# vliu15/3d-brain-tumor-segmentation

Measured on AMD Instinct MI355X. Metric: training volumes/sec (2ch x 128^3), higher is better.
Workload: dtype f32; 1 GPU; BASELINE configs[1]: 2ch x 128^3, batch 1 per GPU, fp32, full fwd+bwd with Dice+KL+L2 VAE loss + Dice metric + TF-form Adam; CLI-default model (base_filters=32, depth=4, groups=8, reduction=8; 42,174,773 params); parallelism=dp1, global_batch=1

## Files before the change

3d-brain-tumor-segmentation_amd/csrc/conv_igemm.hip:

```cpp
#include <stdlib.h>
#include "common.h"
#include "bts_internal.h"

#define MAXSLOT 8

int bts_prof_on();
void bts_prof_begin(int sym, double flops, hipStream_t stream);
void bts_prof_end(hipStream_t stream);

struct IgemmParams {
  const float* x;
  const float* wp;
  const float* bias;
  float* y;
  int N, Di, Hi, Wi, Cin, ldx;
  int Do, Ho, Wo;
  int Cout, ldy, Npad, KG;
  int ODa, OHa, OWa;
  int os, ooz, ooy, oox;
  int s, loz, loy, lox;
  int IZ, IY, IX;
  int lgTX, lgTY, TZ;
  int ntz, nty, ntx;
  int ntaps, flags;
// ... 943 lines not shown
  if (need > 0 && (ws == nullptr || ws_bytes < need)) return 1;
  p.x = x; p.wp = wp; p.bias = bias; p.y = y; p.ldx = ldx; p.ldy = ldy; p.flags = flags;
  p.part = reinterpret_cast<float*>(ws);
  const long tiles = (long)N * p.ntz * p.nty * p.ntx;
  const int ny = p.Npad / 32;
  const int tileVox = p.IZ * p.IY * p.IX;
  const size_t shmem = (size_t)2 * tileVox * 12 * sizeof(float);
  const bool prof = bts_prof_on();
  if (prof) bts_prof_begin(20, 2.0 * 27.0 * Cin * Cout * (double)N * Di * Hi * Wi, stream);
  (void)hipGetLastError(); hipLaunchKernelGGL(upm_kernel, dim3((unsigned)tiles, ny, p.ksplit), dim3(256), shmem, stream, p);
  if (prof) bts_prof_end(stream);
  BTS_LAUNCH_CHECK();
  if (p.ksplit > 1) {
    const long nvox = (long)N * 8 * Di * Hi * Wi;
    long blocks = (nvox * Cout + 255) / 256;
    if (blocks > 4096) blocks = 4096;
    (void)hipGetLastError(); hipLaunchKernelGGL(igemm_reduce_kernel, dim3((int)blocks), dim3(256), 0, stream, p.part, bias, y, nvox, Cout, p.Npad, ldy,
                       p.ksplit, flags);
    BTS_LAUNCH_CHECK();
  }
  return BTS_OK;
}

struct K1sParams {
  const float* x;
  const float* wp;
  const float* bias;
  float* y;
  long nvox;
  int Cin, ldx, Cout, ldy, Npad, KG, flags;
};
template <int NS>
__global__ __launch_bounds__(256, 4) void k1s_kernel(const K1sParams p) {
  const int lane = threadIdx.x & 63;
  const int wave = __builtin_amdgcn_readfirstlane(threadIdx.x >> 6);
  const int h = lane >> 5, l32 = lane & 31;
  const long v0 = (long)blockIdx.x * 256 + wave * 64;
  const float* xrow[2];
#pragma unroll
  for (int ms = 0; ms < 2; ++ms) {
    long v = v0 + ms * 32 + l32;
    if (v >= p.nvox) v = p.nvox - 1;
    xrow[ms] = p.x + v * p.ldx + h * 4;
  }
  int woff[NS];
#pragma unroll
  for (int ns = 0; ns < NS; ++ns) {
    int ncol = (blockIdx.y * NS + ns) * 32 + l32;
    if (ncol >= p.Npad) ncol = p.Npad - 1;
    woff[ns] = (h * p.Npad + ncol) * 4;
  }
  const int wstepKG = 2 * p.Npad * 4;
  f32x16 acc[2][NS];
#pragma unroll
  for (int ms = 0; ms < 2; ++ms)
#pragma unroll
    for (int ns = 0; ns < NS; ++ns)
#pragma unroll
      for (int r = 0; r < 16; ++r) acc[ms][ns][r] = 0.f;
  constexpr int U = (NS == 1) ? 2 : 1;
  f32x4 b[2][U][2], a[2][U][NS];
  auto load = [&](int buf, int kg) {
#pragma unroll
    for (int u = 0; u < U; ++u) {
      const int k = (kg + u < p.KG) ? kg + u : p.KG - 1;
#pragma unroll
      for (int ms = 0; ms < 2; ++ms) b[buf][u][ms] = *reinterpret_cast<const f32x4*>(xrow[ms] + k * 8);
#pragma unroll
      for (int ns = 0; ns < NS; ++ns) a[buf][u][ns] = *reinterpret_cast<const f32x4*>((p.wp + k * wstepKG) + woff[ns]);
    }
  };
  auto mma = [&](int buf, int kg) {
#pragma unroll
    for (int u = 0; u < U; ++u) {
      if (kg + u < p.KG) {
#pragma unroll
        for (int j = 0; j < 4; ++j)
#pragma unroll
          for (int ms = 0; ms < 2; ++ms)
#pragma unroll
            for (int ns = 0; ns < NS; ++ns)
              acc[ms][ns] = __builtin_amdgcn_mfma_f32_32x32x2f32(a[buf][u][ns][j], b[buf][u][ms][j], acc[ms][ns], 0, 0, 0);
      }
    }
  };
  load(0, 0);
  for (int kg = 0; kg < p.KG; kg += 2 * U) {
    if (kg + U < p.KG) load(1, kg + U);
    mma(0, kg);
    if (kg + U < p.KG) {
      if (kg + 2 * U < p.KG) load(0, kg + 2 * U);
      mma(1, kg + U);
    }
  }
#pragma unroll
  for (int ms = 0; ms < 2; ++ms) {
    const long v = v0 + ms * 32 + l32;
    if (v >= p.nvox) continue;
    float* yrow = p.y + v * p.ldy;
#pragma unroll
    for (int ns = 0; ns < NS; ++ns) {
      const int nb = (blockIdx.y * NS + ns) * 32;
#pragma unroll
      for (int g = 0; g < 4; ++g) {
        const int co = nb + 8 * g + 4 * h;
        if (co >= p.Cout) continue;
        f32x4 val = {acc[ms][ns][4 * g + 0], acc[ms][ns][4 * g + 1], acc[ms][ns][4 * g + 2], acc[ms][ns][4 * g + 3]};
        if (p.flags & IG_FLAG_BIAS) {
#pragma unroll
          for (int j = 0; j < 4; ++j)
            if (co + j < p.Cout) val[j] += p.bias[co + j];
        }
        if (p.flags & IG_FLAG_SIGMOID) {
#pragma unroll
          for (int j = 0; j < 4; ++j) val[j] = sigmoidf_(val[j]);
        }
        if ((p.flags & IG_FLAG_VECOUT) && co + 3 < p.Cout) {
          f32x4* dst = reinterpret_cast<f32x4*>(yrow + co);
          if (p.flags & IG_FLAG_ACCUM) val += *dst;
          *dst = val;
        } else {
#pragma unroll
          for (int j = 0; j < 4; ++j)
            if (co + j < p.Cout) yrow[co + j] = (p.flags & IG_FLAG_ACCUM) ? yrow[co + j] + val[j] : val[j];
        }
      }
    }
  }
}

static int launch_k1s(const float* x, const float* wp, const float* bias, float* y, long nvox, int Cin, int ldx, int Cout, int ldy,
                      int flags, hipStream_t stream) {
  if ((Cin & 7) || (ldx & 3) || (((uintptr_t)x) & 15)) return 1;
  const long min_vox = getenv("BTS_IGEMM_K1S_MIN") ? atol(getenv("BTS_IGEMM_K1S_MIN")) : 256 * 256;
  if (nvox < min_vox) return 1;
  K1sParams p;
  p.x = x; p.wp = wp; p.bias = bias; p.y = y; p.nvox = nvox;
  p.Cin = Cin; p.ldx = ldx; p.Cout = Cout; p.ldy = ldy; p.Npad = npad32(Cout); p.KG = Cin / 8;
  p.flags = flags & (IG_FLAG_BIAS | IG_FLAG_ACCUM | IG_FLAG_SIGMOID);
  if ((ldy % 4 == 0) && (((uintptr_t)y) % 16 == 0)) p.flags |= IG_FLAG_VECOUT;
  const long gx = (nvox + 255) / 256;
  if (gx > 0x7fffffffL) return 1;
  const bool prof = bts_prof_on();
  const int ns = (p.Npad >= 64) ? 2 : 1;
  if (prof) bts_prof_begin(21, 2.0 * Cin * (double)Cout * (double)nvox, stream);
  (void)hipGetLastError();
  if (ns == 2) hipLaunchKernelGGL(k1s_kernel<2>, dim3((unsigned)gx, (p.Npad + 63) / 64), dim3(256), 0, stream, p);
  else hipLaunchKernelGGL(k1s_kernel<1>, dim3((unsigned)gx, 1), dim3(256), 0, stream, p);
  if (prof) bts_prof_end(stream);
  BTS_LAUNCH_CHECK();
  return BTS_OK;
}

struct DscParams {
  const float* x;
  const float* wp;
  const float* bias;
  float* y;
  int N, D, H, W, Cin, ldx, Cout, ldy, Npad, KG, ntx, nty, ntz, flags;
};
template <int CO>
__global__ __launch_bounds__(256, 4) void dsc_kernel(const DscParams p) {
  constexpr int S = 12, TX = 32, TY = 4, TZ = 2, IX = TX + 2, IY = TY + 2, IZ = TZ + 2;
  constexpr int tileVox = IZ * IY * IX, nslots = tileVox * 2, NSL = (nslots + 255) / 256;
  __shared__ __attribute__((aligned(16))) float lds[tileVox * S];
  const int tid = threadIdx.x;
  int b = blockIdx.x;
  const int tx = b % p.ntx; b /= p.ntx;
  const int ty = b % p.nty; b /= p.nty;
  const int tz = b % p.ntz;
  const int n = b / p.ntz;
  const int iz0 = tz * TZ - 1, iy0 = ty * TY - 1, ix0 = tx * TX - 1;
  const float* xbase = p.x + ((((long)n * p.D + iz0) * p.H + iy0) * p.W + ix0) * (long)p.ldx;
  int goff[NSL];
#pragma unroll
  for (int i = 0; i < NSL; ++i) {
    const int e = tid + i * 256;
    goff[i] = -1;
    if (e < nslots) {
      const int vox = e >> 1, q = e & 1;
      const int vz = vox / (IY * IX), r = vox - vz * (IY * IX), vy = r / IX, vx = r - vy * IX;
      if ((unsigned)(iz0 + vz) < (unsigned)p.D && (unsigned)(iy0 + vy) < (unsigned)p.H && (unsigned)(ix0 + vx) < (unsigned)p.W)
        goff[i] = ((vz * p.H + vy) * p.W + vx) * p.ldx + q * 4;
    }
  }
  const int mx = tid & (TX - 1), my = (tid >> 5) & (TY - 1), mz = tid >> 7;
  const float* lb = lds + ((mz * IY + my) * IX + mx) * S;
  float acc[CO];
#pragma unroll
  for (int c = 0; c < CO; ++c) acc[c] = 0.f;
  const int wstepKG = 2 * p.Npad * 4, wstepTap = p.KG * wstepKG;
  f32x4 pre[NSL];
  auto fetch = [&](int kg) {
#pragma unroll
    for (int i = 0; i < NSL; ++i) {
      f32x4 v = {0.f, 0.f, 0.f, 0.f};
      if (goff[i] >= 0) v = *reinterpret_cast<const f32x4*>(xbase + goff[i] + kg * 8);
      pre[i] = v;
    }
  };
  fetch(0);
  for (int kg = 0; kg < p.KG; ++kg) {
    __syncthreads();
#pragma unroll
    for (int i = 0; i < NSL; ++i) {
      const int e = tid + i * 256;
      if (e < nslots) *reinterpret_cast<f32x4*>(lds + (e >> 1) * S + (e & 1) * 4) = pre[i];
    }
    __syncthreads();
    if (kg + 1 < p.KG) fetch(kg + 1);
    const float* wk = p.wp + kg * wstepKG;
#pragma unroll
    for (int r = 0; r < 9; ++r) {
      float w[3][2][CO * 4];
#pragma unroll
      for (int dx = 0; dx < 3; ++dx)
#pragma unroll
        for (int hh = 0; hh < 2; ++hh)
#pragma unroll
          for (int q = 0; q < CO * 4; ++q) w[dx][hh][q] = wk[(r * 3 + dx) * wstepTap + hh * p.Npad * 4 + q];
      f32x4 xv[3][2];
#pragma unroll
      for (int dx = 0; dx < 3; ++dx) {
        const float* src = lb + (((r / 3) * IY + r % 3) * IX + dx) * S;
        xv[dx][0] = *reinterpret_cast<const f32x4*>(src);
        xv[dx][1] = *reinterpret_cast<const f32x4*>(src + 4);
      }
      __builtin_amdgcn_sched_barrier(0);
#pragma unroll
      for (int dx = 0; dx < 3; ++dx)
#pragma unroll
        for (int hh = 0; hh < 2; ++hh)
#pragma unroll
          for (int c = 0; c < CO; ++c)
#pragma unroll
            for (int j = 0; j < 4; ++j) acc[c] = fmaf(xv[dx][hh][j], w[dx][hh][c * 4 + j], acc[c]);
      __builtin_amdgcn_sched_barrier(0);
    }
  }
  const int oz = tz * TZ + mz, oy = ty * TY + my, ox = tx * TX + mx;
  if (oz >= p.D || oy >= p.H || ox >= p.W) return;
  float* yrow = p.y + ((((long)n * p.D + oz) * p.H + oy) * p.W + ox) * (long)p.ldy;
#pragma unroll
  for (int c = 0; c < CO; ++c) {
    if (c < p.Cout) {
      float v = acc[c];
      if (p.flags & IG_FLAG_BIAS) v += p.bias[c];
      if (p.flags & IG_FLAG_SIGMOID) v = sigmoidf_(v);
      if (p.flags & IG_FLAG_ACCUM) v += yrow[c];
      yrow[c] = v;
    }
  }
}

static int launch_dsc(const float* x, const float* wp, const float* bias, float* y, int N, int D, int H, int W, int Cin, int ldx,
                      int Cout, int ldy, int flags, hipStream_t stream) {
  if (Cout > 4 || (Cin & 7) || (ldx & 3) || (((uintptr_t)x) & 15)) return 1;
  const long tiles = (long)N * ((D + 1) / 2) * ((H + 3) / 4) * ((W + 31) / 32);
  const long min_tiles = getenv("BTS_IGEMM_DSC_MIN") ? atol(getenv("BTS_IGEMM_DSC_MIN")) : 1024;
  if (tiles < min_tiles || tiles > 0x7fffffffL) return 1;
  DscParams p;
  p.x = x; p.wp = wp; p.bias = bias; p.y = y;
  p.N = N; p.D = D; p.H = H; p.W = W; p.Cin = Cin; p.ldx = ldx; p.Cout = Cout; p.ldy = ldy;
  p.Npad = npad32(Cout); p.KG = Cin / 8;
  p.ntx = (W + 31) / 32; p.nty = (H + 3) / 4; p.ntz = (D + 1) / 2;
  p.flags = flags & (IG_FLAG_BIAS | IG_FLAG_ACCUM | IG_FLAG_SIGMOID);
  const bool prof = bts_prof_on();
  if (prof) bts_prof_begin(22, 2.0 * 27.0 * Cin * (double)Cout * (double)N * D * H * W, stream);
  (void)hipGetLastError();
  if (Cout <= 2) hipLaunchKernelGGL(dsc_kernel<2>, dim3((unsigned)tiles), dim3(256), 0, stream, p);
  else hipLaunchKernelGGL(dsc_kernel<4>, dim3((unsigned)tiles), dim3(256), 0, stream, p);
  if (prof) bts_prof_end(stream);
  BTS_LAUNCH_CHECK();
  return BTS_OK;
}

struct C2Params {
  const float* x;
  const float* wp;
  const float* bias;
  float* y;
  const float* wp2;
  const float* bias2;
  float* y2;
  int N, D, H, W, ldx, Cout, ldy, ldy2, Npad;
  int ntz, nty, ntx;
  double* gnp;
  int gn_G, gn_zt;
};

template <bool F2>
__global__ __launch_bounds__(256, 2) void c2_kernel(const C2Params p) {
  __shared__ float lds[2 * 6 * 6 * 34 + 16];
  const int tid = threadIdx.x;
  const int lane = tid & 63;
  const int wave = __builtin_amdgcn_readfirstlane(tid >> 6);
  const int h = lane >> 5, l32 = lane & 31;
  int b = blockIdx.x;
  const int tx = b % p.ntx; b /= p.ntx;
  const int ty = b % p.nty; b /= p.nty;
  const int tz = b % p.ntz;
  const int n = b / p.ntz;
  const int oz0 = tz * 4, oy0 = ty * 4, ox0 = tx * 32;
  for (int e = tid; e < 6 * 6 * 34; e += 256) {
    const int vz = e / (6 * 34), r = e - vz * (6 * 34);
    const int vy = r / 34, vx = r - vy * 34;
    const int z = oz0 - 1 + vz, yy = oy0 - 1 + vy, xx = ox0 - 1 + vx;
    float v0 = 0.f, v1 = 0.f;
    if ((unsigned)z < (unsigned)p.D && (unsigned)yy < (unsigned)p.H && (unsigned)xx < (unsigned)p.W) {
      const float* s = p.x + ((((long)n * p.D + z) * p.H + yy) * p.W + xx) * (long)p.ldx;
      v0 = s[0]; v1 = s[1];
    }
    lds[e] = v0;
    lds[6 * 6 * 34 + e] = v1;
  }
  float wt[27];
#pragma unroll
  for (int t = 0; t < 27; ++t) wt[t] = p.wp[((long)t * 2 * p.Npad + l32) * 4 + h];
  float w2 = 0.f;
  if (F2) w2 = p.wp2[l32 * 4 + h];
  __syncthreads();
  f32x16 acc[4], acc2[F2 ? 4 : 1];
#pragma unroll
  for (int i = 0; i < 4; ++i)
#pragma unroll
    for (int r = 0; r < 16; ++r) { acc[i][r] = 0.f; if (F2) acc2[F2 ? i : 0][r] = 0.f; }
  const float* lb = lds + h * (6 * 6 * 34) + (wave * 6) * 34 + l32;
#pragma unroll
  for (int kz = 0; kz < 3; ++kz) {
    float f[6][3];
#pragma unroll
    for (int yr = 0; yr < 6; ++yr)
#pragma unroll
      for (int kx = 0; kx < 3; ++kx) f[yr][kx] = lb[(kz * 6 + yr) * 34 + kx];
#pragma unroll
    for (int ky = 0; ky < 3; ++ky)
#pragma unroll
      for (int kx = 0; kx < 3; ++kx)
#pragma unroll
        for (int oy = 0; oy < 4; ++oy)
          acc[oy] = __builtin_amdgcn_mfma_f32_32x32x2f32(wt[(kz * 3 + ky) * 3 + kx], f[oy + ky][kx], acc[oy], 0, 0, 0);
    if (F2 && kz == 1) {
#pragma unroll
      for (int oy = 0; oy < 4; ++oy) acc2[F2 ? oy : 0] = __builtin_amdgcn_mfma_f32_32x32x2f32(w2, f[oy + 1][1], acc2[F2 ? oy : 0], 0, 0, 0);
    }
  }
  const int oz = oz0 + wave, ox = ox0 + l32;
  float gn_s = 0.f, gn_q = 0.f;
  if (oz < p.D && ox < p.W) {
#pragma unroll
    for (int oy = 0; oy < 4; ++oy) {
      const int y = oy0 + oy;
      if (y >= p.H) continue;
      const long pix = (((long)n * p.D + oz) * p.H + y) * p.W + ox;
#pragma unroll
      for (int g = 0; g < 4; ++g) {
        const int co = 8 * g + 4 * h;
        if (co >= p.Cout) continue;
        f32x4 v = {acc[oy][4 * g], acc[oy][4 * g + 1], acc[oy][4 * g + 2], acc[oy][4 * g + 3]};
        if (p.bias) {
#pragma unroll
          for (int j = 0; j < 4; ++j) v[j] += p.bias[co + j];
        }
        if (p.gnp) {
#pragma unroll
          for (int j = 0; j < 4; ++j) { gn_s += v[j]; gn_q = fmaf(v[j], v[j], gn_q); }
        }
        *reinterpret_cast<f32x4*>(p.y + pix * p.ldy + co) = v;
        if (F2) {
          f32x4 v2 = {acc2[F2 ? oy : 0][4 * g], acc2[F2 ? oy : 0][4 * g + 1], acc2[F2 ? oy : 0][4 * g + 2], acc2[F2 ? oy : 0][4 * g + 3]};
          if (p.bias2) {
#pragma unroll
            for (int j = 0; j < 4; ++j) v2[j] += p.bias2[co + j];
          }
          *reinterpret_cast<f32x4*>(p.y2 + pix * p.ldy2 + co) = v2;
        }
      }
    }
  }
  if (p.gnp) {
    const double ds = wave_sum_f64((double)gn_s), dq = wave_sum_f64((double)gn_q);
    __syncthreads();
    double* sh = reinterpret_cast<double*>(lds);
    if (lane == 0) { sh[wave * 2] = ds; sh[wave * 2 + 1] = dq; }
    __syncthreads();
    if (tid == 0) {
      const int g = tz / p.gn_zt;
      const long B = (long)p.gn_zt * p.nty * p.ntx;
      const long b_ = ((long)(tz - g * p.gn_zt) * p.nty + ty) * p.ntx + tx;
      double* o = p.gnp + (((long)n * p.gn_G + g) * B + b_) * 2;
      o[0] = sh[0] + sh[2] + sh[4] + sh[6];
      o[1] = sh[1] + sh[3] + sh[5] + sh[7];
    }
  }
}

static int launch_c2(const float* x, const float* wp, const float* bias, float* y, int N, int D, int H, int W, int Cin, int ldx,
                     int Cout, int ldy, int flags, const float* wp2, const float* bias2, float* y2, int ldy2, double* gnp, int gnG,
                     long* gn_B, hipStream_t stream) {
  if (Cin != 2 || Cout > 32 || Cout % 4 != 0 || ldy % 4 != 0 || (((uintptr_t)y) & 15)) return 1;
  if (flags & (IG_FLAG_ACCUM | IG_FLAG_SIGMOID)) return 1;
  if (y2 != nullptr && (ldy2 % 4 != 0 || (((uintptr_t)y2) & 15))) return 1;
  C2Params p;
  p.x = x; p.wp = wp; p.bias = (flags & IG_FLAG_BIAS) ? bias : nullptr; p.y = y;
  p.wp2 = wp2; p.bias2 = bias2; p.y2 = y2;
  p.N = N; p.D = D; p.H = H; p.W = W; p.ldx = ldx; p.Cout = Cout; p.ldy = ldy; p.ldy2 = ldy2; p.Npad = npad32(Cout);
  p.ntz = (D + 3) / 4; p.nty = (H + 3) / 4; p.ntx = (W + 31) / 32;
  const long tiles = (long)N * p.ntz * p.nty * p.ntx;
  const long min_tiles = getenv("BTS_IGEMM_C2_MIN") ? atol(getenv("BTS_IGEMM_C2_MIN")) : 512;
  if (tiles < min_tiles || tiles > 0x7fffffffL) return 1;
  p.gnp = nullptr; p.gn_G = 0; p.gn_zt = 1;
  if (gnp != nullptr && gnG > 0 && D % gnG == 0 && (D / gnG) % 4 == 0 && getenv("BTS_IGEMM_NOGNFUSE") == nullptr) {
    p.gnp = gnp; p.gn_G = gnG; p.gn_zt = (D / gnG) / 4;
  }
  const bool prof = bts_prof_on();
  if (prof) bts_prof_begin(25, 2.0 * (27.0 + (y2 ? 1.0 : 0.0)) * Cin * (double)Cout * (double)N * D * H * W, stream);
  (void)hipGetLastError();
  if (y2 != nullptr) hipLaunchKernelGGL(c2_kernel<true>, dim3((unsigned)tiles), dim3(256), 0, stream, p);
  else hipLaunchKernelGGL(c2_kernel<false>, dim3((unsigned)tiles), dim3(256), 0, stream, p);
  if (prof) bts_prof_end(stream);
  BTS_LAUNCH_CHECK();
  if (gn_B && p.gnp != nullptr) *gn_B = (long)p.gn_zt * p.nty * p.ntx;
  return BTS_OK;
}

enum Geo { GEO_K1 = 0, GEO_S1 = 1, GEO_DOWN = 2, GEO_UP = 3 };

template <int MS, int NS, int WM, int WN, int KGS, bool FUSE2 = false, bool FIXG = false, bool T27 = false>
static int launch_cfg(IgemmParams& p, hipStream_t stream) {
  constexpr int S = KGS * 8 + 4;
  const int tileVox = p.IZ * p.IY * p.IX;
  if (tileVox * KGS * 2 > 256 * MAXSLOT) return BTS_ERR_SHAPE;
  const int nstages_all = (p.KG + KGS - 1) / KGS;
  const size_t shmem = (size_t)((nstages_all > 1 && !IG_TRI(MS, NS, KGS, FUSE2, FIXG)) ? 2 : 1) * tileVox * S * sizeof(float);
  auto kern = igemm_kernel<MS, NS, WM, WN, KGS, FUSE2, FIXG, T27>;
  static bool attr_done = false;
  if (!attr_done && !p.plan_only) {
    hipError_t e = hipFuncSetAttribute(reinterpret_cast<const void*>(kern), hipFuncAttributeMaxDynamicSharedMemorySize, 160 * 1024);
    if (e != hipSuccess) return (int)e;
    attr_done = true;
  }
  const int NT = 32 * NS * WN;
  dim3 grid(p.N * p.ntz * p.nty * p.ntx, (p.Npad + NT - 1) / NT, p.ncls > 1 ? p.ncls : 1);
  p.ksplit = 1;
  p.kg_per = p.KG;
  p.ws_need = 0;
  const long wgs = (long)grid.x * grid.y;
  const long sk_below = (KGS == 1) ? 512 : 192, sk_target = (KGS == 1) ? 512 : 384;
  if (!FUSE2 && p.ncls <= 1 && wgs < sk_below && p.KG >= 4 * KGS) {
    int ks = (int)((sk_target + wgs - 1) / wgs);
    const int maxks = p.KG / (2 * KGS);
    if (ks > maxks) ks = maxks;
    if (ks > 64) ks = 64;
    if (ks > 1) {
      int per = (p.KG + ks - 1) / ks;
      per = (per + KGS - 1) / KGS * KGS;
      ks = (p.KG + per - 1) / per;
      const long need = (long)ks * p.N * p.Do * p.Ho * p.Wo * p.Npad * 4;
      if (ks > 1 && (p.plan_only || (p.part != nullptr && p.ws_bytes >= need))) {
        p.ksplit = ks;
        p.kg_per = per;
        p.ws_need = need;
        grid.z = ks;
      }
    }
  }
  if (p.ksplit > 1) p.gnp = nullptr;
  p.gn_gridy = (int)grid.y;
  if (p.plan_only) return BTS_OK;
  const bool prof = bts_prof_on();
  if (prof) {
    constexpr int cfgid = (MS == 2 && NS == 1) ? 0 : (MS == 2 && NS == 2) ? 1 : (MS == 1 && NS == 2) ? 2 : (WN == 2) ? 3 : 4;
    const double taps = (p.ncls > 1) ? 27.0 : (double)p.ntaps;
    bts_prof_begin(cfgid + (KGS == 4 ? 8 : 0), 2.0 * taps * p.Cin * p.Cout * (double)p.N * p.Do * p.Ho * p.Wo, stream);
  }
  (void)hipGetLastError(); hipLaunchKernelGGL(kern, grid, dim3(256), shmem, stream, p);
  if (prof) bts_prof_end(stream);
  BTS_LAUNCH_CHECK();
  if (p.ksplit > 1) {
    const long nvox = (long)p.N * p.Do * p.Ho * p.Wo;
    long blocks = (nvox * p.Cout + 255) / 256;
    if (blocks > 4096) blocks = 4096;
    (void)hipGetLastError(); hipLaunchKernelGGL(igemm_reduce_kernel, dim3((int)blocks), dim3(256), 0, stream, p.part, p.bias, p.y, nvox, p.Cout,
                       p.Npad, p.ldy, p.ksplit, p.flags);
    BTS_LAUNCH_CHECK();
  }
  return BTS_OK;
}

static int ilog2(int v) { int l = 0; while ((1 << l) < v) ++l; return l; }

static int choose_cfg(int geo, int N, int Do, int Ho, int Wo, int Npad, int* Mout) {
  const long vox = (long)Do * Ho * Wo;
  int M, cfg;
  if (geo == GEO_DOWN) {
    M = 64;
    cfg = (Npad >= 128) ? 2 : 3;
  } else {
    const long wg256 = (long)N * ((vox + 255) / 256) * ((Npad + 63) / 64);
    if (Npad <= 32) {
      if ((long)N * ((vox + 255) / 256) >= 512) { M = 256; cfg = 0; }
      else { M = 128; cfg = 4; }
    } else if (wg256 >= 512) { M = 256; cfg = 1; }
    else {
      M = 64;
      const long wg64_128 = (long)N * ((vox + 63) / 64) * ((Npad + 127) / 128);
      cfg = (Npad >= 128 && wg64_128 >= 384) ? 2 : 3;
    }
  }
  *Mout = M;
  return cfg;
}

static int launch_igemm(int geo, const float* x, const float* wp, const float* bias, float* y, int N, int Di, int Hi,
                        int Wi, int Cin, int ldx, int Do, int Ho, int Wo, int Cout, int ldy, int ODa, int OHa, int OWa,
                        int pz, int py, int px, int flags, hipStream_t stream, void* ws = nullptr, long ws_bytes = 0,
                        long* need_out = nullptr, const float* wp2 = nullptr, const float* bias2 = nullptr,
                        float* y2 = nullptr, int ldy2 = 0, double* gnp = nullptr, int gnG = 0, long* gn_B = nullptr,
                        const float* x2 = nullptr, int ldx2 = 0) {
  if (gn_B) *gn_B = 0;
  if (geo == GEO_S1 && wp2 == nullptr && need_out == nullptr && Cout <= 4) {
    { const int e = bts_img_ensure_(wp, 1u, stream); if (e != BTS_OK) return e; }
    const int r = launch_dsc(x, wp, bias, y, N, Di, Hi, Wi, Cin, ldx, Cout, ldy, flags, stream);
    if (r != 1) { bts_img_mark_used_(wp, 1u); return r; }
  }
  if (geo == GEO_S1 && need_out == nullptr && Cin == 2 && x2 == nullptr && (wp2 == nullptr) == (y2 == nullptr)) {
    { const int e = bts_img_ensure_(wp, 1u, stream); if (e != BTS_OK) return e; }
    const int r = launch_c2(x, wp, bias, y, N, Di, Hi, Wi, Cin, ldx, Cout, ldy, flags, wp2, bias2, y2, ldy2, gnp, gnG, gn_B, stream);
    if (r != 1) { bts_img_mark_used_(wp, 1u); return r; }
  }
  if (geo == GEO_S1 && need_out == nullptr && !(flags & IG_FLAG_SIGMOID)) {
    const long pairs = (long)((Cin + 7) / 8) * 2 * npad32(Cout) * 4;
    const float* up = wp + 27L * pairs;
    int r = bts_w3_launch_(x, up + 48L * pairs, (flags & IG_FLAG_BIAS) ? bias : nullptr, y, N, Di, Hi, Wi, Cin, ldx, Cout, ldy,
                           (flags & IG_FLAG_ACCUM) ? 1 : 0, gnp, gnG, gn_B, ws, ws_bytes, stream);
    if (r == 1)
      r = bts_wino_launch_(x, up, (flags & IG_FLAG_BIAS) ? bias : nullptr, y, N, Di, Hi, Wi, Cin, ldx, Cout, ldy,
                           (flags & IG_FLAG_ACCUM) ? 1 : 0, gnp, gnG, gn_B, ws, ws_bytes, stream);
    if (r == BTS_OK) {
      if (y2 != nullptr)
        return launch_igemm(GEO_K1, x, wp2, bias2, y2, N, Di, Hi, Wi, Cin, ldx, Di, Hi, Wi, Cout, ldy2, Di, Hi, Wi, 0, 0, 0,
                            bias2 ? IG_FLAG_BIAS : 0, stream);
      if (x2 != nullptr)
        return launch_igemm(GEO_K1, x2, wp2, nullptr, y, N, Di, Hi, Wi, Cin, ldx2, Di, Hi, Wi, Cout, ldy, Di, Hi, Wi, 0, 0, 0,
                            IG_FLAG_ACCUM, stream);
      return BTS_OK;
    }
    if (r != 1) return r;
  }
  if (geo == GEO_K1 && wp2 == nullptr && need_out == nullptr) {
    const int r = launch_k1s(x, wp, bias, y, (long)N * Di * Hi * Wi, Cin, ldx, Cout, ldy, flags, stream);
    if (r != 1) return r;
  }
  if (geo == GEO_UP && pz < 0 && wp2 == nullptr && !(flags & ~(IG_FLAG_BIAS | IG_FLAG_ACCUM | IG_FLAG_SIGMOID | IG_FLAG_VECIN | IG_FLAG_VECOUT))) {
    if (need_out != nullptr) {
      UpmParams pp;
      long need = 0;
      if (plan_upm(pp, N, Di, Hi, Wi, Cin, Cout, &need) && need > 0) { *need_out = need; return BTS_OK; }
    } else {
      const int r = launch_upm(x, wp, bias, y, N, Di, Hi, Wi, Cin, ldx, Cout, ldy, flags, ws, ws_bytes, stream);
      if (r != 1) return r;
    }
  }
  if (geo == GEO_S1 && need_out == nullptr) {
    const int e = bts_img_note_use_(wp, 1u, stream);
    if (e != BTS_OK) return e;
  }
  IgemmParams p;
  p.wp2 = wp2; p.bias2 = bias2; p.y2 = y2; p.ldy2 = ldy2;
  p.x2 = x2; p.ldx2 = ldx2;
  p.part = reinterpret_cast<float*>(ws);
  p.ws_bytes = ws_bytes;
  p.plan_only = need_out != nullptr;
  p.ws_need = 0;
  p.x = x; p.wp = wp; p.bias = bias; p.y = y;
  p.N = N; p.Di = Di; p.Hi = Hi; p.Wi = Wi; p.Cin = Cin; p.ldx = ldx;
  p.Do = Do; p.Ho = Ho; p.Wo = Wo; p.Cout = Cout; p.ldy = ldy;
  p.Npad = npad32(Cout); p.KG = (Cin + 7) / 8;
  p.ODa = ODa; p.OHa = OHa; p.OWa = OWa;
  p.os = 1; p.ooz = p.ooy = p.oox = 0;
  p.s = 1;
  p.flags = flags;
  if ((ldx % 4 == 0) && (Cin % 4 == 0) && (((uintptr_t)x) % 16 == 0)) p.flags |= IG_FLAG_VECIN;
  if ((ldy % 4 == 0) && (Cout % 4 == 0) && (((uintptr_t)y) % 16 == 0)) p.flags |= IG_FLAG_VECOUT;

  int offz[27], offy[27], offx[27], tw[27], nt = 0;
  int lo[3] = {0, 0, 0}, hi[3] = {0, 0, 0};
  if (geo == GEO_K1) {
    offz[0] = offy[0] = offx[0] = 0; tw[0] = 0; nt = 1;
  } else if (geo == GEO_S1) {
    for (int t = 0; t < 27; ++t) { offz[t] = t / 9 - 1; offy[t] = (t / 3) % 3 - 1; offx[t] = t % 3 - 1; tw[t] = t; }
    nt = 27;
    lo[0] = lo[1] = lo[2] = -1; hi[0] = hi[1] = hi[2] = 1;
  } else if (geo == GEO_DOWN) {
    for (int t = 0; t < 27; ++t) { offz[t] = t / 9; offy[t] = (t / 3) % 3; offx[t] = t % 3; tw[t] = t; }
    nt = 27;
    hi[0] = hi[1] = hi[2] = 2;
    p.s = 2;
  } else if (pz < 0) {
    lo[0] = lo[1] = lo[2] = -1;
    p.os = 2;
    nt = 8;
  } else {
    const int par[3] = {pz, py, px};
    int kz[2], ky[2], kx[2], dz[2], dy[2], dx[2], nz, ny, nx;
    auto axis = [](int pp, int* k, int* d) {
      if (pp == 0) { k[0] = 0; d[0] = 0; k[1] = 2; d[1] = -1; return 2; }
      k[0] = 1; d[0] = 0; return 1;
    };
    nz = axis(par[0], kz, dz); ny = axis(par[1], ky, dy); nx = axis(par[2], kx, dx);
    for (int a = 0; a < nz; ++a)
      for (int bb = 0; bb < ny; ++bb)
        for (int c = 0; c < nx; ++c) {
          offz[nt] = dz[a]; offy[nt] = dy[bb]; offx[nt] = dx[c];
          tw[nt] = (kz[a] * 3 + ky[bb]) * 3 + kx[c];
          ++nt;
        }
    lo[0] = par[0] == 0 ? -1 : 0; lo[1] = par[1] == 0 ? -1 : 0; lo[2] = par[2] == 0 ? -1 : 0;
    p.os = 2; p.ooz = pz; p.ooy = py; p.oox = px;
  }
  p.ntaps = nt;
  p.ncls = 1;
  p.loz = lo[0]; p.loy = lo[1]; p.lox = lo[2];

  const int k1 = (geo == GEO_K1);
  int M;
  int cfg = choose_cfg(geo, (geo == GEO_UP && pz < 0) ? 8 * N : N, Do, Ho, Wo, p.Npad, &M);
  int TX = 32;
  while (TX > 4 && TX / 2 >= Wo) TX /= 2;
  if (geo == GEO_DOWN && TX > 8) TX = 8;
  if (TX > M) TX = M;
  int TY = 4;
  while (TY > 1 && TY / 2 >= Ho) TY /= 2;
  if (TX * TY > M) TY = M / TX;
  int TZ = M / (TX * TY);
  while (TZ > 1 && TZ / 2 >= Do && TY * 2 <= 64) { TZ /= 2; TY *= 2; }
  p.lgTX = ilog2(TX); p.lgTY = ilog2(TY); p.TZ = TZ;
  p.ntx = (Wo + TX - 1) / TX; p.nty = (Ho + TY - 1) / TY; p.ntz = (Do + TZ - 1) / TZ;
  p.gnp = nullptr; p.gn_G = 0; p.gn_zt = 1; p.gn_gridy = 1;
  if (gnp != nullptr && gnG > 0 && geo != GEO_UP && Do % gnG == 0 && (Do / gnG) % TZ == 0 && getenv("BTS_IGEMM_NOGNFUSE") == nullptr) {
    p.gnp = gnp; p.gn_G = gnG; p.gn_zt = (Do / gnG) / TZ;
  }
  p.IX = (TX - 1) * p.s + (hi[2] - lo[2] + 1);
  p.IY = (TY - 1) * p.s + (hi[1] - lo[1] + 1);
  p.IZ = (TZ - 1) * p.s + (hi[0] - lo[0] + 1);
  const int KGS = k1 ? 4 : 1;
  const int S = KGS * 8 + 4;
  for (int t = 0; t < nt; ++t) {
    p.tap_lds[t] = (((offz[t] - lo[0]) * p.IY + (offy[t] - lo[1])) * p.IX + (offx[t] - lo[2])) * S;
    p.tap_w[t] = tw[t];
  }
  for (int t = nt; t < 27; ++t) { p.tap_lds[t] = 0; p.tap_w[t] = 0; }
  p.tap_sz = p.IY * p.IX * S; p.tap_sy = p.IX * S; p.tap_sx = S;
  if (geo == GEO_UP && pz < 0) {
    p.ncls = 8;
    for (int c = 0; c < 8; ++c) {
      const int par[3] = {(c >> 2) & 1, (c >> 1) & 1, c & 1};
      int k[3][2], d[3][2], n[3];
      for (int a = 0; a < 3; ++a) {
        if (par[a] == 0) { k[a][0] = 0; d[a][0] = 0; k[a][1] = 2; d[a][1] = -1; n[a] = 2; }
        else { k[a][0] = 1; d[a][0] = 0; n[a] = 1; }
      }
      int ct = 0;
      for (int a = 0; a < n[0]; ++a)
        for (int bb = 0; bb < n[1]; ++bb)
          for (int cc = 0; cc < n[2]; ++cc) {
            p.cls_tl[c][ct] = (((d[0][a] + 1) * p.IY + (d[1][bb] + 1)) * p.IX + (d[2][cc] + 1)) * S;
            p.cls_tw[c][ct] = (k[0][a] * 3 + k[1][bb]) * 3 + k[2][cc];
            ++ct;
          }
      p.cls_nt[c] = ct;
      for (; ct < 8; ++ct) { p.cls_tl[c][ct] = 0; p.cls_tw[c][ct] = 0; }
    }
  }

  int rc;
  const bool fixg = (geo == GEO_S1) && p.IX == 34 && p.IY == 6;
  if (fixg && !k1 && (cfg == 0 || cfg == 1)) {
    if (p.y2 != nullptr) {
      if (cfg == 0) rc = launch_cfg<2, 1, 4, 1, 1, true, true>(p, stream);
      else rc = BTS_ERR_UNSUPPORTED;
    } else {
// ... 248 lines not shown
```

Measured before the change: 27.18 volumes/s.

## Register-block small-Cout direct conv over y rows and transpose F2 c2 MFMA outputs

Reworks the small-Cout direct 3x3x3 conv kernel so each thread computes four y-outputs. Input rows loaded from LDS are reused across the ky taps, LDS padding is dropped, and FMAs use packed two-wide vector form with split accumulators. Tiles grow to 32x8x4, occupancy drops to 2 blocks, and the tile threshold is lowered, so more layers qualify. The fused two-output c2 kernel swaps MFMA operands so lanes map to output channels, which changes its store pattern to scalar per-channel writes. Acceptance checks are moved into predicate functions so the dispatcher commits to a path once it is accepted.

```diff
diff --git a/3d-brain-tumor-segmentation_amd/csrc/conv_igemm.hip b/3d-brain-tumor-segmentation_amd/csrc/conv_igemm.hip
--- a/3d-brain-tumor-segmentation_amd/csrc/conv_igemm.hip
+++ b/3d-brain-tumor-segmentation_amd/csrc/conv_igemm.hip
@@ -1119,6 +1119,11 @@
   return BTS_OK;
 }
 
+typedef float dsc_f32x2 __attribute__((ext_vector_type(2)));
+#define DSC_TX 32
+#define DSC_TY 8
+#define DSC_TZ 4
+#define DSC_YB 4
 struct DscParams {
   const float* x;
   const float* wp;
@@ -1127,10 +1132,11 @@
   int N, D, H, W, Cin, ldx, Cout, ldy, Npad, KG, ntx, nty, ntz, flags;
 };
 template <int CO>
-__global__ __launch_bounds__(256, 4) void dsc_kernel(const DscParams p) {
-  constexpr int S = 12, TX = 32, TY = 4, TZ = 2, IX = TX + 2, IY = TY + 2, IZ = TZ + 2;
+__global__ __launch_bounds__(256, 2) void dsc_kernel(const DscParams p) {
+  constexpr int TX = DSC_TX, TY = DSC_TY, TZ = DSC_TZ, YB = DSC_YB, IX = TX + 2, IY = TY + 2, IZ = TZ + 2;
   constexpr int tileVox = IZ * IY * IX, nslots = tileVox * 2, NSL = (nslots + 255) / 256;
-  __shared__ __attribute__((aligned(16))) float lds[tileVox * S];
+  static_assert(TX == 32 && TY == 2 * YB && TZ == 4, "lane map: x = lane & 31, (z, y block) = tid >> 5");
+  __shared__ __attribute__((aligned(16))) float lds[tileVox * 8];
   const int tid = threadIdx.x;
   int b = blockIdx.x;
   const int tx = b % p.ntx; b /= p.ntx;
@@ -1151,12 +1157,14 @@
         goff[i] = ((vz * p.H + vy) * p.W + vx) * p.ldx + q * 4;
     }
   }
-  const int mx = tid & (TX - 1), my = (tid >> 5) & (TY - 1), mz = tid >> 7;
-  const float* lb = lds + ((mz * IY + my) * IX + mx) * S;
-  float acc[CO];
-#pragma unroll
-  for (int c = 0; c < CO; ++c) acc[c] = 0.f;
-  const int wstepKG = 2 * p.Npad * 4, wstepTap = p.KG * wstepKG;
+  const int mx = tid & (TX - 1), col = tid >> 5, mz = col >> 1, my0 = (col & 1) * YB;
+  const float* lb = lds + ((mz * IY + my0) * IX + mx) * 8;
+  dsc_f32x2 acc[YB][CO];
+#pragma unroll
+  for (int o = 0; o < YB; ++o)
+#pragma unroll
+    for (int c = 0; c < CO; ++c) acc[o][c] = dsc_f32x2{0.f, 0.f};
+  const int wstepKG = 2 * p.Npad * 4, wstepTap = p.KG * wstepKG, whalf = p.Npad * 4;
   f32x4 pre[NSL];
   auto fetch = [&](int kg) {
 #pragma unroll
@@ -1172,66 +1180,79 @@
 #pragma unroll
     for (int i = 0; i < NSL; ++i) {
       const int e = tid + i * 256;
-      if (e < nslots) *reinterpret_cast<f32x4*>(lds + (e >> 1) * S + (e & 1) * 4) = pre[i];
+      if (e < nslots) *reinterpret_cast<f32x4*>(lds + e * 4) = pre[i];
     }
     __syncthreads();
     if (kg + 1 < p.KG) fetch(kg + 1);
     const float* wk = p.wp + kg * wstepKG;
 #pragma unroll
-    for (int r = 0; r < 9; ++r) {
-      float w[3][2][CO * 4];
-#pragma unroll
-      for (int dx = 0; dx < 3; ++dx)
-#pragma unroll
-        for (int hh = 0; hh < 2; ++hh)
-#pragma unroll
-          for (int q = 0; q < CO * 4; ++q) w[dx][hh][q] = wk[(r * 3 + dx) * wstepTap + hh * p.Npad * 4 + q];
-      f32x4 xv[3][2];
-#pragma unroll
-      for (int dx = 0; dx < 3; ++dx) {
-        const float* src = lb + (((r / 3) * IY + r % 3) * IX + dx) * S;
-        xv[dx][0] = *reinterpret_cast<const f32x4*>(src);
-        xv[dx][1] = *reinterpret_cast<const f32x4*>(src + 4);
-      }
-      __builtin_amdgcn_sched_barrier(0);
-#pragma unroll
-      for (int dx = 0; dx < 3; ++dx)
-#pragma unroll
-        for (int hh = 0; hh < 2; ++hh)
-#pragma unroll
-          for (int c = 0; c < CO; ++c)
-#pragma unroll
-            for (int j = 0; j < 4; ++j) acc[c] = fmaf(xv[dx][hh][j], w[dx][hh][c * 4 + j], acc[c]);
-      __builtin_amdgcn_sched_barrier(0);
-    }
-  }
-  const int oz = tz * TZ + mz, oy = ty * TY + my, ox = tx * TX + mx;
-  if (oz >= p.D || oy >= p.H || ox >= p.W) return;
-  float* yrow = p.y + ((((long)n * p.D + oz) * p.H + oy) * p.W + ox) * (long)p.ldy;
-#pragma unroll
-  for (int c = 0; c < CO; ++c) {
-    if (c < p.Cout) {
-      float v = acc[c];
-      if (p.flags & IG_FLAG_BIAS) v += p.bias[c];
-      if (p.flags & IG_FLAG_SIGMOID) v = sigmoidf_(v);
-      if (p.flags & IG_FLAG_ACCUM) v += yrow[c];
-      yrow[c] = v;
-    }
-  }
+    for (int kz = 0; kz < 3; ++kz)
+#pragma unroll
+      for (int kx = 0; kx < 3; ++kx) {
+        f32x4 xv[YB + 2][2];
+#pragma unroll
+        for (int r = 0; r < YB + 2; ++r) {
+          const float* src = lb + ((kz * IY + r) * IX + kx) * 8;
+          xv[r][0] = *reinterpret_cast<const f32x4*>(src);
+          xv[r][1] = *reinterpret_cast<const f32x4*>(src + 4);
+        }
+#pragma unroll
+        for (int ky = 0; ky < 3; ++ky) {
+          const float* wt = wk + ((kz * 3 + ky) * 3 + kx) * wstepTap;
+          f32x4 w[2][CO];
+#pragma unroll
+          for (int hh = 0; hh < 2; ++hh)
+#pragma unroll
+            for (int c = 0; c < CO; ++c) w[hh][c] = *reinterpret_cast<const f32x4*>(wt + hh * whalf + c * 4);
+#pragma unroll
+          for (int o = 0; o < YB; ++o)
+#pragma unroll
+            for (int hh = 0; hh < 2; ++hh)
+#pragma unroll
+              for (int c = 0; c < CO; ++c) {
+                acc[o][c] = __builtin_elementwise_fma(xv[o + ky][hh].xy, w[hh][c].xy, acc[o][c]);
+                acc[o][c] = __builtin_elementwise_fma(xv[o + ky][hh].zw, w[hh][c].zw, acc[o][c]);
+              }
+        }
+      }
+  }
+  const int oz = tz * TZ + mz, ox = tx * TX + mx;
+  if (oz >= p.D || ox >= p.W) return;
+#pragma unroll
+  for (int o = 0; o < YB; ++o) {
+    const int oy = ty * TY + my0 + o;
+    if (oy >= p.H) break;
+    float* yrow = p.y + ((((long)n * p.D + oz) * p.H + oy) * p.W + ox) * (long)p.ldy;
+#pragma unroll
+    for (int c = 0; c < CO; ++c) {
+      if (c < p.Cout) {
+        float v = acc[o][c].x + acc[o][c].y;
+        if (p.flags & IG_FLAG_BIAS) v += p.bias[c];
+        if (p.flags & IG_FLAG_SIGMOID) v = sigmoidf_(v);
+        if (p.flags & IG_FLAG_ACCUM) v += yrow[c];
+        yrow[c] = v;
+      }
+    }
+  }
+}
+
+static bool dsc_accepts(const float* x, int N, int D, int H, int W, int Cin, int ldx, int Cout) {
+  if (Cout > 4 || (Cin & 7) || (ldx & 3) || (((uintptr_t)x) & 15)) return false;
+  const long tiles = (long)N * ((D + DSC_TZ - 1) / DSC_TZ) * ((H + DSC_TY - 1) / DSC_TY) * ((W + DSC_TX - 1) / DSC_TX);
+  const long min_tiles = getenv("BTS_IGEMM_DSC_MIN") ? atol(getenv("BTS_IGEMM_DSC_MIN")) : 256;
+  if (tiles < min_tiles || tiles > 0x7fffffffL) return false;
+  return (double)(DSC_TZ + 2) * H * W * ldx < 2.0e9;
 }
 
 static int launch_dsc(const float* x, const float* wp, const float* bias, float* y, int N, int D, int H, int W, int Cin, int ldx,
                       int Cout, int ldy, int flags, hipStream_t stream) {
-  if (Cout > 4 || (Cin & 7) || (ldx & 3) || (((uintptr_t)x) & 15)) return 1;
-  const long tiles = (long)N * ((D + 1) / 2) * ((H + 3) / 4) * ((W + 31) / 32);
-  const long min_tiles = getenv("BTS_IGEMM_DSC_MIN") ? atol(getenv("BTS_IGEMM_DSC_MIN")) : 1024;
-  if (tiles < min_tiles || tiles > 0x7fffffffL) return 1;
   DscParams p;
   p.x = x; p.wp = wp; p.bias = bias; p.y = y;
   p.N = N; p.D = D; p.H = H; p.W = W; p.Cin = Cin; p.ldx = ldx; p.Cout = Cout; p.ldy = ldy;
   p.Npad = npad32(Cout); p.KG = Cin / 8;
-  p.ntx = (W + 31) / 32; p.nty = (H + 3) / 4; p.ntz = (D + 1) / 2;
+  p.ntx = (W + DSC_TX - 1) / DSC_TX; p.nty = (H + DSC_TY - 1) / DSC_TY; p.ntz = (D + DSC_TZ - 1) / DSC_TZ;
   p.flags = flags & (IG_FLAG_BIAS | IG_FLAG_ACCUM | IG_FLAG_SIGMOID);
+  const long tiles = (long)N * p.ntz * p.nty * p.ntx;
   const bool prof = bts_prof_on();
   if (prof) bts_prof_begin(22, 2.0 * 27.0 * Cin * (double)Cout * (double)N * D * H * W, stream);
   (void)hipGetLastError();
@@ -1306,41 +1327,61 @@
       for (int kx = 0; kx < 3; ++kx)
 #pragma unroll
         for (int oy = 0; oy < 4; ++oy)
-          acc[oy] = __builtin_amdgcn_mfma_f32_32x32x2f32(wt[(kz * 3 + ky) * 3 + kx], f[oy + ky][kx], acc[oy], 0, 0, 0);
+          acc[oy] = F2 ? __builtin_amdgcn_mfma_f32_32x32x2f32(f[oy + ky][kx], wt[(kz * 3 + ky) * 3 + kx], acc[oy], 0, 0, 0)
+                       : __builtin_amdgcn_mfma_f32_32x32x2f32(wt[(kz * 3 + ky) * 3 + kx], f[oy + ky][kx], acc[oy], 0, 0, 0);
     if (F2 && kz == 1) {
 #pragma unroll
-      for (int oy = 0; oy < 4; ++oy) acc2[F2 ? oy : 0] = __builtin_amdgcn_mfma_f32_32x32x2f32(w2, f[oy + 1][1], acc2[F2 ? oy : 0], 0, 0, 0);
-    }
-  }
-  const int oz = oz0 + wave, ox = ox0 + l32;
+      for (int oy = 0; oy < 4; ++oy) acc2[F2 ? oy : 0] = __builtin_amdgcn_mfma_f32_32x32x2f32(f[oy + 1][1], w2, acc2[F2 ? oy : 0], 0, 0, 0);
+    }
+  }
+  const int oz = oz0 + wave;
   float gn_s = 0.f, gn_q = 0.f;
-  if (oz < p.D && ox < p.W) {
-#pragma unroll
-    for (int oy = 0; oy < 4; ++oy) {
-      const int y = oy0 + oy;
-      if (y >= p.H) continue;
-      const long pix = (((long)n * p.D + oz) * p.H + y) * p.W + ox;
-#pragma unroll
-      for (int g = 0; g < 4; ++g) {
-        const int co = 8 * g + 4 * h;
-        if (co >= p.Cout) continue;
-        f32x4 v = {acc[oy][4 * g], acc[oy][4 * g + 1], acc[oy][4 * g + 2], acc[oy][4 * g + 3]};
-        if (p.bias) {
-#pragma unroll
-          for (int j = 0; j < 4; ++j) v[j] += p.bias[co + j];
+  if constexpr (F2) {
+    const int co = l32;
+    if (oz < p.D && co < p.Cout) {
+      const float bco = p.bias ? p.bias[co] : 0.f;
+      const float bco2 = p.bias2 ? p.bias2[co] : 0.f;
+#pragma unroll
+      for (int oy = 0; oy < 4; ++oy) {
+        const int y = oy0 + oy;
+        if (y >= p.H) continue;
+        const long row = (((long)n * p.D + oz) * p.H + y) * p.W;
+#pragma unroll
+        for (int r = 0; r < 16; ++r) {
+          const int x = ox0 + 8 * (r >> 2) + 4 * h + (r & 3);
+          if (x >= p.W) continue;
+          float v = acc[oy][r];
+          if (p.bias) v += bco;
+          if (p.gnp) { gn_s += v; gn_q = fmaf(v, v, gn_q); }
+          p.y[(row + x) * p.ldy + co] = v;
+          float v2 = acc2[F2 ? oy : 0][r];
+          if (p.bias2) v2 += bco2;
+          p.y2[(row + x) * p.ldy2 + co] = v2;
         }
-        if (p.gnp) {
-#pragma unroll
-          for (int j = 0; j < 4; ++j) { gn_s += v[j]; gn_q = fmaf(v[j], v[j], gn_q); }
-        }
-        *reinterpret_cast<f32x4*>(p.y + pix * p.ldy + co) = v;
-        if (F2) {
-          f32x4 v2 = {acc2[F2 ? oy : 0][4 * g], acc2[F2 ? oy : 0][4 * g + 1], acc2[F2 ? oy : 0][4 * g + 2], acc2[F2 ? oy : 0][4 * g + 3]};
-          if (p.bias2) {
-#pragma unroll
-            for (int j = 0; j < 4; ++j) v2[j] += p.bias2[co + j];
+      }
+    }
+  } else {
+    const int ox = ox0 + l32;
+    if (oz < p.D && ox < p.W) {
+#pragma unroll
+      for (int oy = 0; oy < 4; ++oy) {
+        const int y = oy0 + oy;
+        if (y >= p.H) continue;
+        const long pix = (((long)n * p.D + oz) * p.H + y) * p.W + ox;
+#pragma unroll
+        for (int g = 0; g < 4; ++g) {
+          const int co = 8 * g + 4 * h;
+          if (co >= p.Cout) continue;
+          f32x4 v = {acc[oy][4 * g], acc[oy][4 * g + 1], acc[oy][4 * g + 2], acc[oy][4 * g + 3]};
+          if (p.bias) {
+#pragma unroll
+            for (int j = 0; j < 4; ++j) v[j] += p.bias[co + j];
           }
-          *reinterpret_cast<f32x4*>(p.y2 + pix * p.ldy2 + co) = v2;
+          if (p.gnp) {
+#pragma unroll
+            for (int j = 0; j < 4; ++j) { gn_s += v[j]; gn_q = fmaf(v[j], v[j], gn_q); }
+          }
+          *reinterpret_cast<f32x4*>(p.y + pix * p.ldy + co) = v;
         }
       }
     }
@@ -1362,20 +1403,24 @@
   }
 }
 
+static bool c2_accepts(int N, int D, int H, int W, int Cin, int Cout, const float* y, int ldy, int flags, const float* y2, int ldy2) {
+  if (Cin != 2 || Cout > 32 || Cout % 4 != 0 || ldy % 4 != 0 || (((uintptr_t)y) & 15)) return false;
+  if (flags & (IG_FLAG_ACCUM | IG_FLAG_SIGMOID)) return false;
+  if (y2 != nullptr && (ldy2 % 4 != 0 || (((uintptr_t)y2) & 15))) return false;
+  const long tiles = (long)N * ((D + 3) / 4) * ((H + 3) / 4) * ((W + 31) / 32);
+  const long min_tiles = getenv("BTS_IGEMM_C2_MIN") ? atol(getenv("BTS_IGEMM_C2_MIN")) : 512;
+  return tiles >= min_tiles && tiles <= 0x7fffffffL;
+}
+
 static int launch_c2(const float* x, const float* wp, const float* bias, float* y, int N, int D, int H, int W, int Cin, int ldx,
                      int Cout, int ldy, int flags, const float* wp2, const float* bias2, float* y2, int ldy2, double* gnp, int gnG,
                      long* gn_B, hipStream_t stream) {
-  if (Cin != 2 || Cout > 32 || Cout % 4 != 0 || ldy % 4 != 0 || (((uintptr_t)y) & 15)) return 1;
-  if (flags & (IG_FLAG_ACCUM | IG_FLAG_SIGMOID)) return 1;
-  if (y2 != nullptr && (ldy2 % 4 != 0 || (((uintptr_t)y2) & 15))) return 1;
   C2Params p;
   p.x = x; p.wp = wp; p.bias = (flags & IG_FLAG_BIAS) ? bias : nullptr; p.y = y;
   p.wp2 = wp2; p.bias2 = bias2; p.y2 = y2;
   p.N = N; p.D = D; p.H = H; p.W = W; p.ldx = ldx; p.Cout = Cout; p.ldy = ldy; p.ldy2 = ldy2; p.Npad = npad32(Cout);
   p.ntz = (D + 3) / 4; p.nty = (H + 3) / 4; p.ntx = (W + 31) / 32;
   const long tiles = (long)N * p.ntz * p.nty * p.ntx;
-  const long min_tiles = getenv("BTS_IGEMM_C2_MIN") ? atol(getenv("BTS_IGEMM_C2_MIN")) : 512;
-  if (tiles < min_tiles || tiles > 0x7fffffffL) return 1;
   p.gnp = nullptr; p.gn_G = 0; p.gn_zt = 1;
   if (gnp != nullptr && gnG > 0 && D % gnG == 0 && (D / gnG) % 4 == 0 && getenv("BTS_IGEMM_NOGNFUSE") == nullptr) {
     p.gnp = gnp; p.gn_G = gnG; p.gn_zt = (D / gnG) / 4;
@@ -1486,15 +1531,18 @@
                         float* y2 = nullptr, int ldy2 = 0, double* gnp = nullptr, int gnG = 0, long* gn_B = nullptr,
                         const float* x2 = nullptr, int ldx2 = 0) {
   if (gn_B) *gn_B = 0;
-  if (geo == GEO_S1 && wp2 == nullptr && need_out == nullptr && Cout <= 4) {
+  if (geo == GEO_S1 && wp2 == nullptr && need_out == nullptr && dsc_accepts(x, N, Di, Hi, Wi, Cin, ldx, Cout)) {
     { const int e = bts_img_ensure_(wp, 1u, stream); if (e != BTS_OK) return e; }
     const int r = launch_dsc(x, wp, bias, y, N, Di, Hi, Wi, Cin, ldx, Cout, ldy, flags, stream);
-    if (r != 1) { bts_img_mark_used_(wp, 1u); return r; }
-  }
-  if (geo == GEO_S1 && need_out == nullptr && Cin == 2 && x2 == nullptr && (wp2 == nullptr) == (y2 == nullptr)) {
+    if (r == BTS_OK) bts_img_mark_used_(wp, 1u);
+    return r;
+  }
+  if (geo == GEO_S1 && need_out == nullptr && x2 == nullptr && (wp2 == nullptr) == (y2 == nullptr) &&
+      c2_accepts(N, Di, Hi, Wi, Cin, Cout, y, ldy, flags, y2, ldy2)) {
     { const int e = bts_img_ensure_(wp, 1u, stream); if (e != BTS_OK) return e; }
     const int r = launch_c2(x, wp, bias, y, N, Di, Hi, Wi, Cin, ldx, Cout, ldy, flags, wp2, bias2, y2, ldy2, gnp, gnG, gn_B, stream);
-    if (r != 1) { bts_img_mark_used_(wp, 1u); return r; }
+    if (r == BTS_OK) bts_img_mark_used_(wp, 1u);
+    return r;
   }
   if (geo == GEO_S1 && need_out == nullptr && !(flags & IG_FLAG_SIGMOID)) {
     const long pairs = (long)((Cin + 7) / 8) * 2 * npad32(Cout) * 4;
```

Result: no change. 27.30 volumes/s (median of 6 runs) (+0.4%).
